# NOAA-OWP/T-Route

Measured on AMD Instinct MI355X. Metric: segment-timesteps/sec, CONUS NHD 2.7M-seg MC, higher is better.
Workload: dtype f32

## Files before the change

include/trmc.h:

```cpp
#ifndef TRMC_H
#define TRMC_H

#include <stddef.h>
#include <stdint.h>

#ifdef __cplusplus
extern "C" {
#endif

#define TRMC_ABI_VERSION 19

typedef enum trmc_status {
    TRMC_OK = 0,
    TRMC_EINVAL = -1,
    TRMC_ECYCLE = -2,
    TRMC_ENODEVICE = -3,
    TRMC_EHIP = -4,
    TRMC_ENOMEM = -5,
    TRMC_ESTATE = -6
} trmc_status;

enum { TRMC_P_DT = 0, TRMC_P_DX, TRMC_P_BW, TRMC_P_TW, TRMC_P_TWCC, TRMC_P_N,
       TRMC_P_NCC, TRMC_P_CS, TRMC_P_S0, TRMC_NPARAM };

// ... 93 lines not shown
                           const uint8_t *cost_hint, int64_t wide_min_rows, int32_t wide_max_levels, int32_t cluster_rows,
                           int64_t *plan_pos_of_row, int32_t *lag_of_row, int32_t *block_of_row, int32_t *wide_levels,
                           int32_t *cluster_levels, int32_t *cluster_blocks);

int trmc_topology_blocks(int64_t nseg, const int64_t *up_ptr, const int64_t *up_idx,
                         const uint8_t *boundary, const uint8_t *cost_hint, int cost_tiers,
                         int64_t *plan_pos_of_row, int32_t *rank_of_row, int32_t *block_rows, int32_t *nblocks);

int trmc_topology_blocks_general(int64_t nseg, const int64_t *up_ptr, const int64_t *up_idx, const uint8_t *boundary,
                                 int32_t stem_min_rows, int64_t *plan_pos_of_row, int32_t *rank_of_row, int32_t *block_rows,
                                 int32_t *nblocks, int32_t *early_blocks, int32_t early_cap, int32_t *nearly);

int trmc_plan_info(const trmc_plan *plan, int64_t *nseg, int64_t *nseg_routed,
                   int32_t *nlevels, int32_t *precision, int32_t *device);
int trmc_plan_lags(const trmc_plan *plan, int32_t *lag_of_row, int32_t *wide_levels, int32_t *cluster_levels);
int trmc_plan_levels(const trmc_plan *plan, int32_t *level_of_row, int64_t *plan_pos_of_row);

int trmc_upload_forcing(trmc_plan *plan, int nsteps, const void *qlat, int64_t nq,
                        const void *q0, const void *boundary_fvd);

int trmc_upload_forcing_packed(trmc_plan *plan, int nsteps, int64_t nq, int64_t nfeat, const int32_t *raw_a,
                               const int32_t *raw_b, const double *pack_a, const double *pack_b,
                               const int64_t *feat_of_row, const void *q0, const void *boundary_fvd);

int trmc_set_boundary_flow_device(trmc_plan *plan, int nsteps, const void *q_dev);

int trmc_set_reservoirs(trmc_plan *plan, int64_t nres, const int64_t *res_rows, const void *par,
                        double routing_period);
int trmc_download_reservoir_inflow(trmc_plan *plan, void *inflow_out);

// ... 114 lines not shown
```

t-route_amd/_lib.py:

```python
import ctypes as C
import os

import numpy as np

_HERE = os.path.dirname(os.path.abspath(__file__))
LIB_PATH = os.environ.get("TRMC_LIB_PATH") or os.path.join(_HERE, "libtrmc.so")

TRMC_OK, TRMC_EINVAL, TRMC_ECYCLE, TRMC_ENODEVICE, TRMC_EHIP, TRMC_ENOMEM, TRMC_ESTATE = 0, -1, -2, -3, -4, -5, -6
ENGINE_AUTO, ENGINE_LEVELS, ENGINE_FLOW, PLAN_SHORT_TS, PLAN_FULL_TS = 0, 1, 2, 4, 8
NPARAM = 9
PARAM_COLS = ("dt", "dx", "bw", "tw", "twcc", "n", "ncc", "cs", "s0")


class Stats(C.Structure):
    _fields_ = [
        ("nseg", C.c_int64), ("nseg_routed", C.c_int64), ("nlevels", C.c_int32), ("nsteps", C.c_int32),
        ("assume_short_ts", C.c_int32), ("main_launches", C.c_int32), ("segment_steps", C.c_int64),
        ("ms_prep", C.c_double), ("ms_main", C.c_double), ("ms_emit", C.c_double), ("ms_total", C.c_double),
        ("wide_levels", C.c_int32), ("wide_k", C.c_int32), ("wide_launches", C.c_int32), ("mid_levels", C.c_int32),
        ("wide_segment_steps", C.c_int64), ("ms_wide", C.c_double), ("mid_k", C.c_int32), ("mid_launches", C.c_int32),
        ("arithmetic", C.c_int32), ("reserved0", C.c_int32),
    ]

    def as_dict(self):
# ... 76 lines not shown
    "trmc_stream_wait": (_int, [_vp, _i64]),
    "trmc_stream_info": (_int, [_vp, _P(_i32), _P(_i32), _P(_i32), _P(_i32), _P(_i32), _P(_i64), _P(_i64), _P(_i64)]),
    "trmc_stream_day_ms": (_int, [_vp, _i64, _P(C.c_double)]),
    "trmc_stream_end": (_int, [_vp]),
    "trmc_plan_arithmetic": (_int, [_vp, _P(_i32)]),
    "trmc_plan_engine": (_int, [_vp, _P(_i32)]),
    "trmc_plan_destroy": (None, [_vp]),
    "trmc_topology_levels": (_int, [_i64, _vp, _vp, _vp, _vp, _vp, _P(_i32)]),
    "trmc_topology_levels_hinted": (_int, [_i64, _vp, _vp, _vp, _vp, _vp, _vp, _P(_i32)]),
    "trmc_topology_clusters": (_int, [_i64, _vp, _vp, _vp, _vp, _i64, _i32, _i32, _vp, _vp, _vp, _P(_i32), _P(_i32), _P(_i32)]),
    "trmc_topology_blocks": (_int, [_i64, _vp, _vp, _vp, _vp, _int, _vp, _vp, _P(_i32), _P(_i32)]),
    "trmc_topology_blocks_general": (_int, [_i64, _vp, _vp, _vp, _i32, _vp, _vp, _P(_i32), _P(_i32), _vp, _i32, _P(_i32)]),
    "trmc_plan_info": (_int, [_vp, _P(_i64), _P(_i64), _P(_i32), _P(_i32), _P(_i32)]),
    "trmc_plan_levels": (_int, [_vp, _vp, _vp]),
    "trmc_plan_lags": (_int, [_vp, _vp, _P(_i32), _P(_i32)]),
    "trmc_upload_forcing": (_int, [_vp, _int, _vp, _i64, _vp, _vp]),
    "trmc_upload_forcing_packed": (_int, [_vp, _int, _i64, _i64, _vp, _vp, _vp, _vp, _vp, _vp, _vp]),
    "trmc_set_boundary_flow_device": (_int, [_vp, _int, _vp]),
    "trmc_set_reservoirs": (_int, [_vp, _i64, _vp, _vp, C.c_double]),
    "trmc_download_reservoir_inflow": (_int, [_vp, _vp]),
    "trmc_set_reservoir_da": (_int, [_vp, _i64, _vp, _vp, _P(ReservoirDaTable), _P(ReservoirDaTable), _P(ReservoirDaTable)]),
    "trmc_download_reservoir_da": (_int, [_vp, _vp, _vp]),
    "trmc_reservoir_da_steps": (_int, [_int, _int, _i64, _i64, _vp, _vp, _vp, _vp, _vp, _vp]),
    "trmc_set_nudging": (_int, [_vp, _int, _i64, _vp, _vp, _vp, _vp]),
    "trmc_set_nudging_successors": (_int, [_vp, C.c_int64, _vp]),
    "trmc_download_nudge": (_int, [_vp, _vp]),
    "trmc_route_device": (_int, [_vp, _int, _int, _int]),
    "trmc_route_begin": (_int, [_vp, _int, _int, _int]),
    "trmc_route_advance": (_int, [_vp, _int]),
    "trmc_route_end": (_int, [_vp]),
# ... 55 lines not shown
    "trmc_event_record": (_int, [_int, _vp, _vp]),
    "trmc_stream_wait_event": (_int, [_int, _vp, _vp]),
}

SIGNATURES_DW = {
    "trdw_last_error": (C.c_char_p, []),
    "trdw_select_device": (_int, [_int]),
    "trdw_diffnw": (_int, [_vp] * 42),
    "trdw_diffnw_batch": (_int, [_int, _vp]),
    "trdw_last_timing": (_int, [_P(C.c_double), _P(C.c_double)]),
    "trdw_configure": (_int, [_vp]),
}

_LIB = None
_HOST_ONLY = {"trmc_last_error", "trmc_abi_version", "trmc_topology_levels", "trmc_topology_levels_hinted", "trmc_topology_blocks", "trmc_topology_clusters",
              "trmc_topology_blocks_general", "trmc_get_stats", "trmc_plan_info", "trmc_plan_levels", "trmc_plan_lags", "trmc_plan_engine",
              "trmc_plan_arithmetic", "trmc_stream_info", "trdw_last_error", "trdw_last_timing", "trdw_configure", "trmc_comm_info"}


class _Marking:

    def __init__(self, cdll):
        self.__dict__["_cdll"] = cdll

    def __getattr__(self, name):
        fn = getattr(self._cdll, name)
        if name in _HOST_ONLY:
            self.__dict__[name] = fn
            return fn

        def call(*args, _fn=fn):
# ... 177 lines not shown
```

t-route_amd/csrc/abi.inc:

```

static void stream_release(trmc_plan *pl);
static bool stream_active(const trmc_plan *pl);

const char *trmc_last_error(void) { return g_err.c_str(); }
int trmc_abi_version(void) { return TRMC_ABI_VERSION; }

int trmc_device_count(int *count)
{
    if (!count) return fail(TRMC_EINVAL, "count is NULL");
    int c = 0;
    hipError_t e = hipGetDeviceCount(&c);
    if (e != hipSuccess) {
        *count = 0;
        return fail(TRMC_ENODEVICE, std::string("hipGetDeviceCount: ") + hipGetErrorString(e));
    }
    *count = c;
    return 0;
}

int trmc_topology_levels(int64_t nseg, const int64_t *up_ptr, const int64_t *up_idx, const uint8_t *boundary,
                         int32_t *level_of_row, int64_t *plan_pos_of_row, int32_t *nlevels)
{
    return trmc_topology_levels_hinted(nseg, up_ptr, up_idx, boundary, nullptr, level_of_row, plan_pos_of_row, nlevels);
}
// ... 6 lines not shown
    const int rc = trmc::build_topology(nseg, up_ptr, up_idx, boundary, t, err, cost_hint);
    if (rc) return fail(rc == -2 ? TRMC_ECYCLE : TRMC_EINVAL, err);
    for (int64_t r = 0; r < nseg; ++r) {
        if (level_of_row) level_of_row[r] = t.level_of_row[r];
        if (plan_pos_of_row) plan_pos_of_row[r] = t.pos_of_row[r];
    }
    if (nlevels) *nlevels = t.nlevels;
    return 0;
}

int trmc_topology_clusters(int64_t nseg, const int64_t *up_ptr, const int64_t *up_idx, const uint8_t *boundary,
                           const uint8_t *cost_hint, int64_t wide_min_rows, int32_t wide_max_levels, int32_t cluster_rows,
                           int64_t *plan_pos_of_row, int32_t *lag_of_row, int32_t *block_of_row, int32_t *wide_levels,
                           int32_t *cluster_levels, int32_t *cluster_blocks)
{
    if (cluster_rows <= 0 || cluster_rows > kTileBlock) return fail(TRMC_EINVAL, "cluster_rows must be in [1, 128]");
    trmc::Topology t;
    std::string err;
    const int rc = trmc::build_topology(nseg, up_ptr, up_idx, boundary, t, err, cost_hint, 0, true, kWideMaxLevels, wide_min_rows,
                                        std::min<int32_t>(wide_max_levels, kWideMaxLevels), 0, 0, 0, cluster_rows);
    if (rc) return fail(rc == -2 ? TRMC_ECYCLE : TRMC_EINVAL, err);
    const int32_t nb = t.ncl > 0 ? (int32_t)t.cblk_ptr.size() - 1 : 0;
    std::vector<int32_t> blk_of_pos((size_t)nseg, -1);
    for (int32_t b = 0; b < nb; ++b)
        for (int32_t p = t.cblk_ptr[(size_t)b]; p < t.cblk_ptr[(size_t)b + 1]; ++p) blk_of_pos[(size_t)p] = b;
    for (int64_t r = 0; r < nseg; ++r) {
        const int32_t p = t.pos_of_row[r];
        if (plan_pos_of_row) plan_pos_of_row[r] = p;
        if (lag_of_row) lag_of_row[r] = t.level_of_row[r] < 0 ? -1 : t.lagk_of_pos[(size_t)p];
        if (block_of_row) block_of_row[r] = blk_of_pos[(size_t)p];
    }
// ... 152 lines not shown
    pl->flow = engine == TRMC_ENGINE_FLOW;
    pl->watchdog_ticks = (uint64_t)(o.flow_watchdog_ms > 0 ? o.flow_watchdog_ms : 30000) * 100000ull;
    {
        int ncu = 256;
        if (hipSetDevice(device) == hipSuccess) (void)hipDeviceGetAttribute(&ncu, hipDeviceAttributeMultiprocessorCount, device);
        trmc_plan::Opt &po = pl->opt;
        po.tol = o.arithmetic == TRMC_ARITH_TOLERANCE;
        po.wide_min_rows = o.wide_min_rows < 0 ? 0 : (o.wide_min_rows > 0 ? o.wide_min_rows : (po.tol ? 256L : 288L) * ncu);
        po.wide_levels = (int32_t)std::min<long>(o.wide_levels > 0 ? o.wide_levels : 16, kWideMaxLevels);
        po.wide_k = o.wide_k > 0 ? o.wide_k : 0;
        po.mid_min_rows = o.mid_min_rows < 0 ? 0 : (o.mid_min_rows > 0 ? o.mid_min_rows : kMidDefaultRowsPerCu * (int64_t)ncu);
        po.mid_levels = (int32_t)std::min<long>(o.mid_levels > 0 ? o.mid_levels : 12, kMidMaxLevels);
        po.mid_k = o.mid_k > 0 ? o.mid_k : 4;
        po.tile_perm_group = o.tile_perm_group < 0 ? 0 : (o.tile_perm_group > 0 ? 1 : -1);
        po.hot_rows = o.hot_rows < 0 ? 0 : (o.hot_rows > 0 ? 1 : -1);
        po.cluster_rows = o.cluster_rows > 0 ? std::min<int32_t>(o.cluster_rows, kTileBlock) : 0;
        po.cluster_late_lag = std::max(0, o.cluster_late_lag);
        po.stream_split = std::max(0, o.stream_split);
        po.hot_wave_rows = std::max(0, std::min(64, o.hot_wave_rows));
        po.velocity_on_demand = o.velocity_on_demand;
        po.sequence = o.sequence_mode != 0;
        po.flow_overlap = o.flow_overlap != 0;
        po.flow_lean = o.flow_lean;
        po.flow_debug = o.flow_debug != 0;
    }
    const bool tiers = (flags & TRMC_PLAN_SHORT_TS) != 0;
    std::string err;
    int64_t wide_min_rows = 0, mid_min_rows = 0;
    int32_t wide_max_levels = 0, mid_max_levels = 0;
    if (tiers && !pl->flow && cost_hint && o.tail_sort >= 0) {
        wide_min_rows = pl->opt.wide_min_rows;
// ... 2 lines not shown
        mid_max_levels = pl->opt.mid_levels;
    }
    int32_t cluster_rows = 0;
    if (tiers && !pl->flow && pl->opt.cluster_rows > 0) {
        cluster_rows = pl->opt.cluster_rows;
        wide_min_rows = pl->opt.wide_min_rows;
        wide_max_levels = pl->opt.wide_levels;
        mid_min_rows = 0;
        mid_max_levels = 0;
        pl->opt.mid_min_rows = 0;
    }
    int32_t stem_min_rows = 0;
    if (pl->flow && (flags & TRMC_PLAN_FULL_TS)) stem_min_rows = o.stem_min_rows < 0 ? 0 : (o.stem_min_rows > 0 ? o.stem_min_rows : 1024);
    const int trc = trmc::build_topology(nseg, up_ptr, up_idx, boundary, pl->topo, err, cost_hint, pl->flow ? kFlowBlock : 0, tiers,
                                         (tiers && !pl->flow) ? kWideMaxLevels : 0, wide_min_rows, wide_max_levels, stem_min_rows,
                                         mid_min_rows, mid_max_levels, cluster_rows, pl->opt.cluster_late_lag);
    if (trc) {
        delete pl;
        return fail(trc == -2 ? TRMC_ECYCLE : TRMC_EINVAL, err);
    }
    pl->device = device;
    pl->hinted = cost_hint != nullptr && (!pl->flow || tiers);
    pl->precision = precision;
    pl->esz = precision == 32 ? 4 : 8;
    pl->nseg = nseg;
    pl->nseg_pad = (nseg + 63) / 64 * 64;
    if (pl->nseg_pad == 0) pl->nseg_pad = 64;
    pl->nrouted = nseg - pl->topo.nboundary;
    pl->dt_uniform = true;
    pl->dt = nseg ? params[TRMC_P_DT] : 0.0;
    for (int64_t r = 1; r < nseg; ++r)
// ... 283 lines not shown
    return 0;
}

int trmc_plan_lags(const trmc_plan *pl, int32_t *lag_of_row, int32_t *wide_levels, int32_t *cluster_levels)
{
    if (!pl) return fail(TRMC_EINVAL, "plan is NULL");
    const trmc::Topology &t = pl->topo;
    if (t.cl_rows <= 0) return fail(TRMC_EINVAL, "the plan is not in cluster order (trmc_plan_options.cluster_rows)");
    for (int64_t r = 0; lag_of_row && r < pl->nseg; ++r)
        lag_of_row[r] = t.level_of_row[r] < 0 ? -1 : t.lagk_of_pos[(size_t)t.pos_of_row[r]];
    if (wide_levels) *wide_levels = t.cl_from_level;
    if (cluster_levels) *cluster_levels = t.ncl;
    return 0;
}

int trmc_plan_levels(const trmc_plan *pl, int32_t *level_of_row, int64_t *plan_pos_of_row)
{
    if (!pl) return fail(TRMC_EINVAL, "plan is NULL");
    for (int64_t r = 0; r < pl->nseg; ++r) {
        if (level_of_row) level_of_row[r] = pl->topo.level_of_row[r];
        if (plan_pos_of_row) plan_pos_of_row[r] = pl->topo.pos_of_row[r];
    }
    return 0;
}

static int final_state_into(trmc_plan *pl, void *dst, int32_t nsteps_of_window)
{
    const int32_t n = (int32_t)pl->nseg, T_ = nsteps_of_window >= 0 ? nsteps_of_window : pl->routed_nsteps;
    const size_t plane = (size_t)(T_ + 1) * pl->nseg_pad;
    const int32_t *rop = (const int32_t *)pl->row_of_pos.p;
// ... 1077 lines not shown
```

t-route_amd/csrc/host_levels.inc:

```

template <class T> T *col(trmc_plan *pl, int c) { return (T *)pl->params.p + (size_t)c * pl->nseg_pad; }

template <class T> int upload_params(trmc_plan *pl, const float *params)
{
    const int64_t n = pl->nseg, np = pl->nseg_pad;
    std::vector<T> host((size_t)TRMC_NPARAM * np, T(0));
    const size_t all_cols = (size_t)kTotalCols * np;
    bool sane = true;
    auto in_range = [](float v) { return v >= 0x1p-14f && v <= 0x1p17f; };
    auto within = [](float v, float lo, float hi) { return v >= lo && v <= hi; };
    for (int64_t p = 0; p < n; ++p) {
        const float *src = params + (size_t)pl->topo.row_of_pos[p] * TRMC_NPARAM;
        for (int c = 0; c < TRMC_NPARAM; ++c) host[(size_t)c * np + p] = (T)src[c];
        const float cs = src[TRMC_P_CS];
        sane = sane && in_range(src[TRMC_P_BW]) && in_range(src[TRMC_P_N]) && (cs == 0.0f || in_range(cs))
               && (src[TRMC_P_TWCC] == 0.0f || in_range(src[TRMC_P_TWCC])) && (src[TRMC_P_NCC] == 0.0f || in_range(src[TRMC_P_NCC]))
               && within(src[TRMC_P_DT], 0x1p-20f, 0x1p40f) && within(src[TRMC_P_DX], 0x1p-10f, 0x1p19f)
               && within(src[TRMC_P_S0], 0x1p-30f, 0x1p10f);
    }
    pl->params_sane = sane && sizeof(T) == 4;
    if (int rc = pl->params.ensure(all_cols * sizeof(T))) return rc;
    HIP_TRY(hipMemcpy(pl->params.p, host.data(), host.size() * sizeof(T), hipMemcpyHostToDevice));
    if (n > 0) {
        hipLaunchKernelGGL((k_make_const<T>), dim3((unsigned)((n + kBlock - 1) / kBlock)), dim3(kBlock), 0, pl->stream,
// ... 146 lines not shown
        }
    }
    if (lazy) {
        if (dec) hipLaunchKernelGGL((k_mc_tile<T, false, true, true>), grid, block, 0, st, a, p0, p1, tile, K);
        else hipLaunchKernelGGL((k_mc_tile<T, false, false, true>), grid, block, 0, st, a, p0, p1, tile, K);
        return;
    }
    if (dec) hipLaunchKernelGGL((k_mc_tile<T, false, true>), grid, block, 0, st, a, p0, p1, tile, K);
    else hipLaunchKernelGGL((k_mc_tile<T, false, false>), grid, block, 0, st, a, p0, p1, tile, K);
}

template <class T>
inline void launch_ctile(hipStream_t st, const StepArgs<T> &a, const int32_t *cblk_ptr, int32_t b0, int32_t b1, int32_t tile, int32_t K,
                         bool tol)
{
    const dim3 grid((unsigned)(b1 - b0)), block(kTileBlock);
    const bool dec = a.dec != nullptr;
    const bool lazy = a.v_every != 0 && !a.out;
    if constexpr (sizeof(T) == 4) {
        if (a.res_da) {
            if (dec) hipLaunchKernelGGL((k_mc_ctile_rda<true>), grid, block, 0, st, a, cblk_ptr, b0, tile, K);
            else hipLaunchKernelGGL((k_mc_ctile_rda<false>), grid, block, 0, st, a, cblk_ptr, b0, tile, K);
            return;
        }
        if (tol) {
            if (lazy) {
                if (dec) hipLaunchKernelGGL((k_mc_ctile<T, true, true, true>), grid, block, 0, st, a, cblk_ptr, b0, tile, K);
                else hipLaunchKernelGGL((k_mc_ctile<T, true, false, true>), grid, block, 0, st, a, cblk_ptr, b0, tile, K);
            } else if (dec) hipLaunchKernelGGL((k_mc_ctile<T, true, true>), grid, block, 0, st, a, cblk_ptr, b0, tile, K);
            else hipLaunchKernelGGL((k_mc_ctile<T, true, false>), grid, block, 0, st, a, cblk_ptr, b0, tile, K);
            return;
// ... 419 lines not shown
```

t-route_amd/csrc/k_mc_ctile.inc:

```
template <class T, bool TOL, bool DEC, bool LAZYV, bool RDA>
__device__ __forceinline__ void mc_ctile_rows(const StepArgs<T> &a, const int32_t *__restrict__ cblk_ptr, int32_t cb0, int32_t tile, int32_t K);
template <class T, bool TOL = false, bool DEC = false, bool LAZYV = false>
__global__ void __launch_bounds__(kTileBlock, sizeof(T) == 4 ? (LAZYV ? TRMC_TILE_WAVES_LAZY : TRMC_TILE_WAVES) : 1)
k_mc_ctile(const StepArgs<T> a, const int32_t *__restrict__ cblk_ptr, const int32_t cb0, const int32_t tile, const int32_t K)
{
    mc_ctile_rows<T, TOL, DEC, LAZYV, false>(a, cblk_ptr, cb0, tile, K);
}
template <bool DEC>
__global__ void __launch_bounds__(kTileBlock, TRMC_TILE_WAVES)
k_mc_ctile_rda(const StepArgs<float> a, const int32_t *__restrict__ cblk_ptr, const int32_t cb0, const int32_t tile, const int32_t K)
{
    mc_ctile_rows<float, false, DEC, false, true>(a, cblk_ptr, cb0, tile, K);
}
template <class T, bool TOL, bool DEC, bool LAZYV, bool RDA>
__device__ __forceinline__ void mc_ctile_rows(const StepArgs<T> &a, const int32_t *__restrict__ cblk_ptr, const int32_t cb0,
                                              const int32_t tile, const int32_t K)
{
    using M = typename DevMath<T, TOL>::type;
    const ColdArgs<StepArgs<T>> cold = cold_args<StepArgs<T>>();
    __shared__ uint64_t s_tab[TRMC_POW_TAB_WORDS];
    __shared__ T s_out[3 * kTileStage * kTileBlock];
    __shared__ T s_x[2 * kTileBlock];
    M m{stage_pow_tables(s_tab), false};
    m.sane = a.sane;

    const int32_t cb = cb0 + (int32_t)blockIdx.x;
    const int32_t lo = cblk_ptr[cb], hi = cblk_ptr[cb + 1];
    int32_t behind, slot, slot_next;
    const bool in_range = seq_locate(a, tile, a.level[lo], behind, slot, slot_next);
    const int32_t t_lo = behind * K + 1, t_hi = min(behind * K + K, a.nsteps);
    if (!in_range || t_lo > t_hi) return;

    int32_t s = lo + (int32_t)threadIdx.x;
    bool active = s < hi;
    if (a.cls_last) {
        const int32_t c = active ? (int32_t)(a.cls_last[s] & 0x7f) : 0x80;
        const int32_t key = (c & 0x80) ? 8 : 7 - min(c, 7);
        bool none;
        s = lo + block_partition_by_class<kTileBlock>(key, none);
        active = !none;
    }
    if (a.cls_last) {
        const int32_t cp = active ? (int32_t)(a.cls_last[s] & 0x7f) : 0;
        if (__any(cp >= 3)) __builtin_amdgcn_s_setprio(3);
        else if (__any(cp == 2)) __builtin_amdgcn_s_setprio(2);
        else __builtin_amdgcn_s_setprio(1);
    } else
        __builtin_amdgcn_s_setprio(2);
    const uint32_t su = (uint32_t)(active ? s : lo);
    const uint32_t sl = su - (uint32_t)lo;
    uint32_t ob = su * (uint32_t)sizeof(T);
    const size_t np = (size_t)a.nseg_pad;
    trmc::ChannelParams<T> p;
    p.dt = a.dt_col ? at(a.dt_col, ob) : a.dt;
// ... 21 lines not shown
    const int32_t in1 = (uy >= lo && uy < hi) ? (uy - lo) * (int32_t)sizeof(T) : -1;
    const int32_t ri = (active && a.res_of_pos) ? a.res_of_pos[su] : -1;
    const int32_t gi = (active && a.gage_of_pos) ? a.gage_of_pos[su] : -1;

    T *const q_tm = a.q_tm + (size_t)slot * (size_t)a.slot_tm;
    const size_t ql_base = (size_t)slot * (size_t)a.slot_qlat;
    T q_prev = at(q_tm + (size_t)(t_lo - 1) * np, ob);
    T d_prev = at(a.d_tm + (size_t)slot * (size_t)a.slot_tm + (size_t)(t_lo - 1) * np, ob);
    T *const out_row = a.out + (size_t)slot * (size_t)a.slot_out + (size_t)a.row_of_pos[su] * (size_t)a.nsteps * 3;
    int32_t ql_col = (t_lo - 1) / a.qts, ql_left = a.qts - (t_lo - 1) % a.qts;
    T ql = at(a.qlat_tm + ql_base + (size_t)ql_col * np, ob);
    m.coef_ok = coef_guard(p.dt, ql);
    const bool count_cost = a.it_sum != nullptr;
    int32_t it_acc = 0, it_last = 0, staged = 0;
    bool over_last = false;
    if (active) s_x[(size_t)((t_lo - 1) & 1) * kTileBlock + sl] = q_prev;
    __syncthreads();
    T *q_up = q_tm + (size_t)(t_lo - 1) * np;
    const int32_t v_every = (LAZYV && DEC) ? cold->v_every : 0;
    int32_t v_left = v_every > 0 ? (v_every - 1) - ((t_lo - 1) % v_every) : 0;
    for (int32_t t = t_lo; t <= t_hi; ++t, q_up += np) {
        bool want_v = false;
        if constexpr (LAZYV && DEC) {
            want_v = v_every > 0 && v_left == 0;
            if (v_every > 0) v_left = v_left == 0 ? v_every - 1 : v_left - 1;
        }
        if (active) {
            if (ql_left == 0) {
                ++ql_col;
                ql = at(cold->qlat_tm + ql_base + (size_t)ql_col * np, ob);
                m.coef_ok = coef_guard(p.dt, ql);
                ql_left = cold->qts;
            }
            --ql_left;
            const T *const sx = s_x + (size_t)((t - 1) & 1) * kTileBlock;
            T qup = T(0);
            if (u.x >= 0) qup += in0 >= 0 ? at(sx, (uint32_t)in0) : at(q_up, (uint32_t)u.x * (uint32_t)sizeof(T));
            if (uy >= 0) qup += in1 >= 0 ? at(sx, (uint32_t)in1) : at(q_up, (uint32_t)uy * (uint32_t)sizeof(T));
            if (uy >= 0) {
                if (u.y & 0x40000000) {
                    const int32_t *const up_ptr = cold->up_ptr, *const up_idx = cold->up_idx;
                    const int32_t k1 = up_ptr[su + 1];
                    for (int32_t k = up_ptr[su] + 2; k < k1; ++k) {
                        const int32_t uk = up_idx[k];
                        qup += (uk >= lo && uk < hi) ? sx[uk - lo] : at(q_up, (uint32_t)uk * (uint32_t)sizeof(T));
                    }
                }
            }
            T q_new, v_new, d_new;
            if (ri >= 0) {
// ... 29 lines not shown
                    const T *const da_a = cold->da_a;
                    const uint8_t mode = cold->da_mode[e];
                    T nudge = T(0);
                    if (mode == 1) {
                        nudge = da_a[e] - q_new;
                        q_new = da_a[e];
                    } else if (mode == 2) {
                        nudge = (da_a[e] - q_new) * cold->da_w[e];
                        q_new = q_new + nudge;
                    }
                    cold->da_nudge[e] = nudge;
                }
            }
            asm volatile("" : "+v"(ob));
            at(q_up + np, ob) = q_new;
            s_x[(size_t)(t & 1) * kTileBlock + sl] = q_new;
            if (t == t_hi) {
                at(cold->d_tm + (size_t)slot * (size_t)cold->slot_tm + (size_t)t * np, ob) = d_new;
                if (cold->seq_slots > 1 && t == cold->nsteps) {
                    at(cold->q_tm + (size_t)slot_next * (size_t)cold->slot_tm, ob) = q_new;
                    at(cold->d_tm + (size_t)slot_next * (size_t)cold->slot_tm, ob) = d_new;
                }
            }
            q_prev = q_new;
            d_prev = d_new;
            if (LAZYV && want_v && it_last > 0) v_new = trmc::step_velocity<T, M>(p, c, d_new, m);
            if (DEC || (!LAZYV && a.out)) {
                T *so = s_out + (size_t)(staged * 3) * kTileBlock + threadIdx.x;
                so[0] = q_new;
                so[kTileBlock] = v_new;
                so[2 * kTileBlock] = d_new;
                ++staged;
                if (staged == kTileStage || t == t_hi) {
                    T *dst = out_row + (size_t)(t - staged) * 3;
                    const T *si = s_out + threadIdx.x;
                    if (LAZYV || !a.out) {
                    } else if (a.out_vec && (staged & 3) == 0) {
                        for (int j = 0; j < 3 * staged / 4; ++j) {
                            float4 v;
                            v.x = (float)si[(4 * j + 0) * kTileBlock];
                            v.y = (float)si[(4 * j + 1) * kTileBlock];
                            v.z = (float)si[(4 * j + 2) * kTileBlock];
                            v.w = (float)si[(4 * j + 3) * kTileBlock];
                            reinterpret_cast<float4 *>(dst)[j] = v;
                        }
                    } else {
                        for (int32_t e = 0; e < 3 * staged; ++e) dst[e] = si[e * kTileBlock];
                    }
                    if constexpr (DEC) {
                        const int32_t ds = cold->dec_stride;
                        for (int32_t k = t / ds; k >= 1 && k * ds > t - staged; --k) {
                            if (k > cold->dec_keep) continue;
                            const int32_t kslot = k * ds - (t - staged) - 1;
                            T *dd = cold->dec + (size_t)slot * (size_t)cold->slot_dec + ((size_t)cold->row_of_pos[su] * (size_t)cold->dec_keep + (size_t)(k - 1)) * 3;
                            dd[0] = si[(kslot * 3 + 0) * kTileBlock];
                            dd[1] = si[(kslot * 3 + 1) * kTileBlock];
                            dd[2] = si[(kslot * 3 + 2) * kTileBlock];
                        }
                    }
                    staged = 0;
                }
            }
        }
        __syncthreads();
    }
    if (!active) return;
    if (t_hi == cold->nsteps) cold->it_prev[su] = (uint8_t)min(it_last, 255);
    if (uint8_t *const cls = cold->cls_last) cls[su] = (uint8_t)(min(it_last, 3) + (over_last ? 4 : 0));
    if (uint16_t *const it_sum = cold->it_sum) it_sum[su] = (uint16_t)min(65535, (int)it_sum[su] + it_acc);
}
```

t-route_amd/csrc/kernels_levels.inc:

```
template <class A> using ColdArgs = const __attribute__((address_space(4))) A *;
template <class A> __device__ __forceinline__ ColdArgs<A> cold_args()
{
    ColdArgs<A> p = (ColdArgs<A>)__builtin_amdgcn_kernarg_segment_ptr();
    asm volatile("" : "+s"(p));
    return p;
}
template <class T> struct StepArgs {
    const T *dx, *bw, *twcc, *n, *ncc, *s0;
    const T *z, *bfd, *sqrt_s0, *sq1pz2, *s0_n, *s0_ncc, *inv_n;
    const T *dt_col;
    T dt;
    const int32_t *up_ptr, *up_idx, *level;
    const int2 *up2;
    const int32_t *lag;
    const T *qlat_tm;
    T *q_tm, *v_tm, *d_tm;
    uint8_t *it_prev;
    uint16_t *it_sum;
    bool sane;
    const int32_t *res_of_pos;
    const T *res_par;
    T *res_inflow;
    T res_dt;
    void *res_da;
// ... 217 lines not shown
    mc_tile_rows<T, TOL, DEC, LAZYV, false>(a, s_begin, s_end, tile, K);
}
template <bool DEC>
__global__ void __launch_bounds__(kTileBlock, TRMC_TILE_WAVES)
k_mc_tile_rda(const StepArgs<float> a, const int32_t s_begin, const int32_t s_end, const int32_t tile, const int32_t K)
{
    mc_tile_rows<float, false, DEC, false, true>(a, s_begin, s_end, tile, K);
}
template <class T, bool TOL, bool DEC, bool LAZYV, bool RDA>
__device__ __forceinline__ void mc_tile_rows(const StepArgs<T> &a, const int32_t s_begin, const int32_t s_end, const int32_t tile,
                                             const int32_t K)
{
    using M = typename DevMath<T, TOL>::type;
    const ColdArgs<StepArgs<T>> cold = cold_args<StepArgs<T>>();
    __shared__ uint64_t s_tab[TRMC_POW_TAB_WORDS];
    __shared__ T s_out[3 * kTileStage * kTileBlock];
    M m{stage_pow_tables(s_tab), false};
    m.sane = a.sane;

    int32_t s;
    bool from_hot = false;
    int32_t *const hot_list = a.cls_last ? cold->hot_list : nullptr;
    const int32_t hot_blocks = hot_list ? cold->hot_home : 0;
    if ((int32_t)blockIdx.x < hot_blocks) {
        const int32_t cur = cold->hot_cur, cap = cold->hot_cap, H = cold->hot_wave_rows;
        const int32_t lane = (int32_t)(threadIdx.x & 63u), wave = (int32_t)blockIdx.x * (kTileBlock / 64) + (int32_t)(threadIdx.x >> 6);
        const int32_t i = wave * H + lane;
        const int32_t nlist = min(cold->hot_cnt[cur], cap);
        if (lane >= H || i >= nlist) return;
        if (lane == 0) atomicAdd(&cold->hot_cnt[3], min(nlist - i, H));
        s = hot_list[(size_t)cur * (size_t)cap + (size_t)i];
// ... 457 lines not shown
```

t-route_amd/csrc/topology.cpp:

```cpp
#include "topology.hpp"

#include <algorithm>
#include <cstdio>
#include <string>
#include <cstdlib>
#include <limits>
#include <utility>

namespace trmc {

int build_topology(int64_t nseg, const int64_t *up_ptr, const int64_t *up_idx,
                   const uint8_t *boundary, Topology &t, std::string &err, const uint8_t *cost_hint, int32_t block_rows,
                   bool cost_tiers, int32_t boundary_floor, int64_t wide_min_rows, int32_t wide_max_levels, int32_t stem_min_rows,
                   int64_t mid_min_rows, int32_t mid_max_levels, int32_t cluster_rows, int32_t cluster_late_lag)
{
    if (nseg < 0 || nseg >= std::numeric_limits<int32_t>::max()) {
        err = "nseg out of range";
        return -1;
    }
    if (nseg > 0 && (!up_ptr || up_ptr[0] != 0)) {
        err = "up_ptr must start at 0";
        return -1;
    }
    const int64_t nnz = nseg ? up_ptr[nseg] : 0;
    for (int64_t r = 0; r < nseg; ++r)
        if (up_ptr[r + 1] < up_ptr[r]) {
            err = "up_ptr is not monotone at row " + std::to_string(r);
            return -1;
        }
// ... 399 lines not shown
            std::stable_sort(idx.begin(), idx.end(), [&](int32_t a, int32_t b) { return key[a] < key[b]; });
            for (int32_t i = 0; i < m; ++i) {
                t.row_of_pos[p0 + i] = rows[idx[i]];
                t.pos_of_row[rows[idx[i]]] = p0 + i;
            }
        }
    }

    if (cluster_rows > 0 && t.nlevels > 0) {
        int32_t W = 0;
        if (wide_min_rows > 0)
            while (W < t.nlevels && W < wide_max_levels && (int64_t)(t.lvl_ptr[W + 1] - t.lvl_ptr[W]) >= wide_min_rows) ++W;
        t.lagk_of_pos.assign(nseg, 0);
        if (W < t.nlevels) {
            const int32_t B = cluster_rows;
            std::vector<int32_t> cl(nseg, -1), root(nseg), size(nseg, 1);
            for (int64_t r = 0; r < nseg; ++r) root[r] = (int32_t)r;
            auto find = [&](int32_t x) {
                while (root[x] != x) {
                    root[x] = root[root[x]];
                    x = root[x];
                }
                return x;
            };
            std::vector<int32_t> tops;
            int32_t maxcl = 0;
            for (const int32_t r : queue) {
                if (t.level_of_row[r] < W) continue;
                int32_t m = -1;
                for (int64_t k = up_ptr[r]; k < up_ptr[r + 1]; ++k) {
// ... 53 lines not shown
            std::vector<std::vector<int32_t>> by_cl((size_t)C);
            for (int32_t c = 0; c < (int32_t)members.size(); ++c) by_cl[(size_t)cl_of[(size_t)c]].push_back(c);
            int32_t p = t.lvl_ptr[W];
            t.cblk_ptr.clear();
            t.cblk_of_cl.assign((size_t)C + 1, 0);
            std::vector<std::vector<int32_t>> bins;
            std::vector<int32_t> fill;
            for (int32_t c = 0; c < C; ++c) {
                std::vector<int32_t> &cs = by_cl[(size_t)c];
                std::stable_sort(cs.begin(), cs.end(), [&](int32_t a, int32_t b) {
                    if (cost_of[(size_t)a] != cost_of[(size_t)b]) return cost_of[(size_t)a] > cost_of[(size_t)b];
                    return members[(size_t)a].size() > members[(size_t)b].size();
                });
                bins.clear();
                fill.clear();
                std::vector<std::vector<int32_t>> by_free((size_t)B + 1);
                for (const int32_t k : cs) {
                    const int32_t n = (int32_t)members[(size_t)k].size();
                    int32_t b = -1;
                    for (int32_t f = n; f <= B && b < 0; ++f)
                        if (!by_free[(size_t)f].empty()) {
                            b = by_free[(size_t)f].back();
                            by_free[(size_t)f].pop_back();
                        }
                    if (b < 0) {
                        b = (int32_t)bins.size();
                        bins.emplace_back();
                        fill.push_back(0);
                    }
                    bins[(size_t)b].push_back(k);
                    fill[(size_t)b] += n;
                    by_free[(size_t)(B - fill[(size_t)b])].push_back(b);
                }
                t.cblk_of_cl[(size_t)c] = (int32_t)t.cblk_ptr.size();
                for (const auto &bin : bins) {
                    t.cblk_ptr.push_back(p);
                    for (const int32_t k : bin)
                        for (const int32_t r : members[(size_t)k]) {
                            t.row_of_pos[p] = r;
                            t.pos_of_row[r] = p;
                            t.lagk_of_pos[p] = W + c;
                            ++p;
                        }
                }
            }
            t.cblk_of_cl[(size_t)C] = (int32_t)t.cblk_ptr.size();
            t.cblk_ptr.push_back(p);
            if (p != t.lvl_ptr[t.nlevels]) {
                err = "internal: the cluster order lost rows";
                return -2;
            }
            t.ncl = C;
            t.tail_from_level = W;
        }
        for (int32_t l = 0; l < W; ++l)
            for (int32_t q = t.lvl_ptr[l]; q < t.lvl_ptr[l + 1]; ++q) t.lagk_of_pos[q] = l;
        t.cl_rows = cluster_rows;
        t.cl_from_level = W;
    } else
    if (cost_hint && wide_min_rows > 0 && wide_max_levels > 0) {
        int32_t W = 0;
        while (W < t.nlevels && W < wide_max_levels && (int64_t)(t.lvl_ptr[W + 1] - t.lvl_ptr[W]) >= wide_min_rows) ++W;
        if (W > 0 && mid_min_rows > 0)
            for (int32_t m = 0; W < t.nlevels && m < mid_max_levels && (int64_t)(t.lvl_ptr[W + 1] - t.lvl_ptr[W]) >= mid_min_rows; ++m) ++W;
        if (W > 0 && W < t.nlevels) {
            const int32_t p0 = t.lvl_ptr[W], p1 = t.lvl_ptr[t.nlevels];
            std::vector<int32_t> rows(t.row_of_pos.begin() + p0, t.row_of_pos.begin() + p1);
            std::stable_sort(rows.begin(), rows.end(), [&](int32_t a, int32_t b) { return cost_hint[a] > cost_hint[b]; });
            for (int32_t i = 0; i < p1 - p0; ++i) {
                t.row_of_pos[p0 + i] = rows[i];
                t.pos_of_row[rows[i]] = p0 + i;
            }
// ... 10 lines not shown
```

t-route_amd/csrc/topology.hpp:

```cpp
#pragma once
#include <cstdint>
#include <string>
#include <vector>

namespace trmc {

struct Topology {
    int64_t nseg = 0;
    int64_t nboundary = 0;
    int32_t nlevels = 0;
    std::vector<int32_t> level_of_row;
    std::vector<int32_t> pos_of_row;
    std::vector<int32_t> row_of_pos;
    std::vector<int32_t> lvl_ptr;
    int32_t tail_from_level = 0;
    std::vector<int32_t> up_ptr;
    std::vector<int32_t> up_idx;
    std::vector<int32_t> boundary_rows;
    int32_t block_rows = 0;
    int32_t nblocks = 0;
    std::vector<int32_t> rank_of_pos;
    int32_t maxrank = 0;
    std::vector<uint8_t> cost_of_wave;
    std::vector<uint8_t> prio_of_wave;
    std::vector<int32_t> early_blocks;
    int32_t cl_rows = 0;
    int32_t cl_from_level = 0;
    int32_t ncl = 0;
    std::vector<int32_t> cblk_ptr;
    std::vector<int32_t> cblk_of_cl;
    std::vector<int32_t> lagk_of_pos;
};

int build_topology(int64_t nseg, const int64_t *up_ptr, const int64_t *up_idx,
                   const uint8_t *boundary, Topology &topo, std::string &err, const uint8_t *cost_hint = nullptr,
                   int32_t block_rows = 0, bool cost_tiers = true, int32_t boundary_floor = 0, int64_t wide_min_rows = 0,
                   int32_t wide_max_levels = 0, int32_t stem_min_rows = 0, int64_t mid_min_rows = 0, int32_t mid_max_levels = 0,
                   int32_t cluster_rows = 0, int32_t cluster_late_lag = 0);

}
```

t-route_amd/plan.py:

```python
import ctypes as C
import os

import numpy as np

from . import _lib


def csr_from_lists(lists):
    ptr = np.zeros(len(lists) + 1, dtype=np.int64)
    if lists:
        ptr[1:] = np.cumsum([len(x) for x in lists])
    idx = np.fromiter((v for x in lists for v in x), dtype=np.int64, count=int(ptr[-1]))
    return ptr, idx


def topology_levels(up_ptr, up_idx, boundary=None, cost_hint=None):
    up_ptr = np.ascontiguousarray(up_ptr, dtype=np.int64)
    up_idx = np.ascontiguousarray(up_idx, dtype=np.int64)
    nseg = up_ptr.shape[0] - 1
    b = None if boundary is None else np.ascontiguousarray(boundary, dtype=np.uint8)
    lvl = np.empty(nseg, dtype=np.int32)
    pos = np.empty(nseg, dtype=np.int64)
    nl = C.c_int32(0)
    h = None if cost_hint is None else np.ascontiguousarray(cost_hint, dtype=np.uint8)
# ... 116 lines not shown
        return {"nseg": nseg.value, "nseg_routed": nr.value, "nlevels": nl.value, "precision": pr.value,
                "device": dev.value}

    def levels(self):
        lvl = np.empty(self.nseg, dtype=np.int32)
        pos = np.empty(self.nseg, dtype=np.int64)
        _lib.check(_lib.lib().trmc_plan_levels(self._h, _lib.ptr(lvl), _lib.ptr(pos)))
        return lvl, pos

    def lags(self):
        lag = np.empty(self.nseg, dtype=np.int32)
        w, c = C.c_int32(0), C.c_int32(0)
        _lib.check(_lib.lib().trmc_plan_lags(self._h, _lib.ptr(lag), C.byref(w), C.byref(c)))
        return lag, w.value, c.value

    def stats(self):
        s = _lib.Stats()
        _lib.check(_lib.lib().trmc_get_stats(self._h, C.byref(s)))
        return s.as_dict()

    def upload_forcing(self, nsteps, qlat, q0, boundary_fvd=None):
        qlat = np.ascontiguousarray(qlat, dtype=self.dtype)
        if qlat.ndim != 2 or qlat.shape[0] != self.nseg:
            raise ValueError(f"Number of rows in Qlat is incorrect: expected ({self.nseg}), got ({qlat.shape[0]})")
        if q0 is not None:
            q0 = np.ascontiguousarray(q0, dtype=self.dtype)
            if q0.shape != (self.nseg, 3):
                raise ValueError("initial_conditions shape mismatch")
        bf = None
        if self.nboundary and boundary_fvd is not None:
# ... 409 lines not shown
```

Measured before the change: 61.76 billion.

## Widen cluster-tile workgroups to pack multiple clusters per block

Decouples the cluster-tile kernel's workgroup size from the generic tile block size. The new size defaults to 512 threads, so the bin packer in topology can place several clusters (each up to 128 rows) into one workgroup. The aim is fewer, fuller blocks and fewer wasted lanes across the cluster-ordered levels. The shared-memory staging depth is halved above 512 threads, and the output staging buffer shrinks to one element when unused (lazy-velocity without decimation). Larger workgroups may lower occupancy and raise barrier cost. A host query for the per-row cluster block assignment is also added.

```diff
diff --git a/include/trmc.h b/include/trmc.h
--- a/include/trmc.h
+++ b/include/trmc.h
@@ -131,6 +131,7 @@
 int trmc_plan_info(const trmc_plan *plan, int64_t *nseg, int64_t *nseg_routed,
                    int32_t *nlevels, int32_t *precision, int32_t *device);
 int trmc_plan_lags(const trmc_plan *plan, int32_t *lag_of_row, int32_t *wide_levels, int32_t *cluster_levels);
+int trmc_plan_cluster_blocks(const trmc_plan *plan, int32_t *block_of_row, int32_t *block_width, int32_t *cluster_blocks);
 int trmc_plan_levels(const trmc_plan *plan, int32_t *level_of_row, int64_t *plan_pos_of_row);
 
 int trmc_upload_forcing(trmc_plan *plan, int nsteps, const void *qlat, int64_t nq,
diff --git a/t-route_amd/_lib.py b/t-route_amd/_lib.py
--- a/t-route_amd/_lib.py
+++ b/t-route_amd/_lib.py
@@ -114,6 +114,7 @@
     "trmc_plan_info": (_int, [_vp, _P(_i64), _P(_i64), _P(_i32), _P(_i32), _P(_i32)]),
     "trmc_plan_levels": (_int, [_vp, _vp, _vp]),
     "trmc_plan_lags": (_int, [_vp, _vp, _P(_i32), _P(_i32)]),
+    "trmc_plan_cluster_blocks": (_int, [_vp, _vp, _P(_i32), _P(_i32)]),
     "trmc_upload_forcing": (_int, [_vp, _int, _vp, _i64, _vp, _vp]),
     "trmc_upload_forcing_packed": (_int, [_vp, _int, _i64, _i64, _vp, _vp, _vp, _vp, _vp, _vp, _vp]),
     "trmc_set_boundary_flow_device": (_int, [_vp, _int, _vp]),
@@ -199,7 +200,7 @@
 
 _LIB = None
 _HOST_ONLY = {"trmc_last_error", "trmc_abi_version", "trmc_topology_levels", "trmc_topology_levels_hinted", "trmc_topology_blocks", "trmc_topology_clusters",
-              "trmc_topology_blocks_general", "trmc_get_stats", "trmc_plan_info", "trmc_plan_levels", "trmc_plan_lags", "trmc_plan_engine",
+              "trmc_topology_blocks_general", "trmc_get_stats", "trmc_plan_info", "trmc_plan_levels", "trmc_plan_lags", "trmc_plan_cluster_blocks", "trmc_plan_engine",
               "trmc_plan_arithmetic", "trmc_stream_info", "trdw_last_error", "trdw_last_timing", "trdw_configure", "trmc_comm_info"}
 
 
diff --git a/t-route_amd/csrc/abi.inc b/t-route_amd/csrc/abi.inc
--- a/t-route_amd/csrc/abi.inc
+++ b/t-route_amd/csrc/abi.inc
@@ -44,7 +44,7 @@
                            int64_t *plan_pos_of_row, int32_t *lag_of_row, int32_t *block_of_row, int32_t *wide_levels,
                            int32_t *cluster_levels, int32_t *cluster_blocks)
 {
-    if (cluster_rows <= 0 || cluster_rows > kTileBlock) return fail(TRMC_EINVAL, "cluster_rows must be in [1, 128]");
+    if (cluster_rows <= 0 || cluster_rows > kClusterRowsMax) return fail(TRMC_EINVAL, "cluster_rows must be in [1, 128]");
     trmc::Topology t;
     std::string err;
     const int rc = trmc::build_topology(nseg, up_ptr, up_idx, boundary, t, err, cost_hint, 0, true, kWideMaxLevels, wide_min_rows,
@@ -227,7 +227,7 @@
         po.mid_k = o.mid_k > 0 ? o.mid_k : 4;
         po.tile_perm_group = o.tile_perm_group < 0 ? 0 : (o.tile_perm_group > 0 ? 1 : -1);
         po.hot_rows = o.hot_rows < 0 ? 0 : (o.hot_rows > 0 ? 1 : -1);
-        po.cluster_rows = o.cluster_rows > 0 ? std::min<int32_t>(o.cluster_rows, kTileBlock) : 0;
+        po.cluster_rows = o.cluster_rows > 0 ? std::min<int32_t>(o.cluster_rows, kClusterRowsMax) : 0;
         po.cluster_late_lag = std::max(0, o.cluster_late_lag);
         po.stream_split = std::max(0, o.stream_split);
         po.hot_wave_rows = std::max(0, std::min(64, o.hot_wave_rows));
@@ -260,7 +260,7 @@
     if (pl->flow && (flags & TRMC_PLAN_FULL_TS)) stem_min_rows = o.stem_min_rows < 0 ? 0 : (o.stem_min_rows > 0 ? o.stem_min_rows : 1024);
     const int trc = trmc::build_topology(nseg, up_ptr, up_idx, boundary, pl->topo, err, cost_hint, pl->flow ? kFlowBlock : 0, tiers,
                                          (tiers && !pl->flow) ? kWideMaxLevels : 0, wide_min_rows, wide_max_levels, stem_min_rows,
-                                         mid_min_rows, mid_max_levels, cluster_rows, pl->opt.cluster_late_lag);
+                                         mid_min_rows, mid_max_levels, cluster_rows, pl->opt.cluster_late_lag, kCtileBlock);
     if (trc) {
         delete pl;
         return fail(trc == -2 ? TRMC_ECYCLE : TRMC_EINVAL, err);
@@ -574,6 +574,22 @@
     return 0;
 }
 
+int trmc_plan_cluster_blocks(const trmc_plan *pl, int32_t *block_of_row, int32_t *block_width, int32_t *cluster_blocks)
+{
+    if (!pl) return fail(TRMC_EINVAL, "plan is NULL");
+    const trmc::Topology &t = pl->topo;
+    if (t.cl_rows <= 0) return fail(TRMC_EINVAL, "the plan is not in cluster order (trmc_plan_options.cluster_rows)");
+    const int32_t nb = t.ncl > 0 ? (int32_t)t.cblk_ptr.size() - 1 : 0;
+    if (block_of_row) {
+        for (int64_t r = 0; r < pl->nseg; ++r) block_of_row[r] = -1;
+        for (int32_t b = 0; b < nb; ++b)
+            for (int32_t p = t.cblk_ptr[(size_t)b]; p < t.cblk_ptr[(size_t)b + 1]; ++p) block_of_row[t.row_of_pos[(size_t)p]] = b;
+    }
+    if (block_width) *block_width = kCtileBlock;
+    if (cluster_blocks) *cluster_blocks = nb;
+    return 0;
+}
+
 int trmc_plan_levels(const trmc_plan *pl, int32_t *level_of_row, int64_t *plan_pos_of_row)
 {
     if (!pl) return fail(TRMC_EINVAL, "plan is NULL");
diff --git a/t-route_amd/csrc/host_levels.inc b/t-route_amd/csrc/host_levels.inc
--- a/t-route_amd/csrc/host_levels.inc
+++ b/t-route_amd/csrc/host_levels.inc
@@ -184,7 +184,7 @@
 inline void launch_ctile(hipStream_t st, const StepArgs<T> &a, const int32_t *cblk_ptr, int32_t b0, int32_t b1, int32_t tile, int32_t K,
                          bool tol)
 {
-    const dim3 grid((unsigned)(b1 - b0)), block(kTileBlock);
+    const dim3 grid((unsigned)(b1 - b0)), block(kCtileBlock);
     const bool dec = a.dec != nullptr;
     const bool lazy = a.v_every != 0 && !a.out;
     if constexpr (sizeof(T) == 4) {
diff --git a/t-route_amd/csrc/k_mc_ctile.inc b/t-route_amd/csrc/k_mc_ctile.inc
--- a/t-route_amd/csrc/k_mc_ctile.inc
+++ b/t-route_amd/csrc/k_mc_ctile.inc
@@ -1,13 +1,21 @@
+#ifndef TRMC_CTILE_BLOCK
+#define TRMC_CTILE_BLOCK 512
+#endif
+constexpr int kCtileBlock = TRMC_CTILE_BLOCK;
+constexpr int kClusterRowsMax = 128;
+static_assert(kCtileBlock % 64 == 0 && kCtileBlock >= kClusterRowsMax && kCtileBlock <= 1024,
+              "TRMC_CTILE_BLOCK: whole wavefronts, at least one cluster, at most one workgroup");
+constexpr int kCtileStage = kCtileBlock > 512 ? kTileStage / 2 : kTileStage;
 template <class T, bool TOL, bool DEC, bool LAZYV, bool RDA>
 __device__ __forceinline__ void mc_ctile_rows(const StepArgs<T> &a, const int32_t *__restrict__ cblk_ptr, int32_t cb0, int32_t tile, int32_t K);
 template <class T, bool TOL = false, bool DEC = false, bool LAZYV = false>
-__global__ void __launch_bounds__(kTileBlock, sizeof(T) == 4 ? (LAZYV ? TRMC_TILE_WAVES_LAZY : TRMC_TILE_WAVES) : 1)
+__global__ void __launch_bounds__(kCtileBlock, sizeof(T) == 4 ? (LAZYV ? TRMC_TILE_WAVES_LAZY : TRMC_TILE_WAVES) : 1)
 k_mc_ctile(const StepArgs<T> a, const int32_t *__restrict__ cblk_ptr, const int32_t cb0, const int32_t tile, const int32_t K)
 {
     mc_ctile_rows<T, TOL, DEC, LAZYV, false>(a, cblk_ptr, cb0, tile, K);
 }
 template <bool DEC>
-__global__ void __launch_bounds__(kTileBlock, TRMC_TILE_WAVES)
+__global__ void __launch_bounds__(kCtileBlock, TRMC_TILE_WAVES)
 k_mc_ctile_rda(const StepArgs<float> a, const int32_t *__restrict__ cblk_ptr, const int32_t cb0, const int32_t tile, const int32_t K)
 {
     mc_ctile_rows<float, false, DEC, false, true>(a, cblk_ptr, cb0, tile, K);
@@ -19,8 +27,8 @@
     using M = typename DevMath<T, TOL>::type;
     const ColdArgs<StepArgs<T>> cold = cold_args<StepArgs<T>>();
     __shared__ uint64_t s_tab[TRMC_POW_TAB_WORDS];
-    __shared__ T s_out[3 * kTileStage * kTileBlock];
-    __shared__ T s_x[2 * kTileBlock];
+    __shared__ T s_out[(DEC || !LAZYV) ? 3 * kCtileStage * kCtileBlock : 1];
+    __shared__ T s_x[2 * kCtileBlock];
     M m{stage_pow_tables(s_tab), false};
     m.sane = a.sane;
 
@@ -37,7 +45,7 @@
         const int32_t c = active ? (int32_t)(a.cls_last[s] & 0x7f) : 0x80;
         const int32_t key = (c & 0x80) ? 8 : 7 - min(c, 7);
         bool none;
-        s = lo + block_partition_by_class<kTileBlock>(key, none);
+        s = lo + block_partition_by_class<kCtileBlock>(key, none);
         active = !none;
     }
     if (a.cls_last) {
@@ -89,7 +97,7 @@
     const bool count_cost = a.it_sum != nullptr;
     int32_t it_acc = 0, it_last = 0, staged = 0;
     bool over_last = false;
-    if (active) s_x[(size_t)((t_lo - 1) & 1) * kTileBlock + sl] = q_prev;
+    if (active) s_x[(size_t)((t_lo - 1) & 1) * kCtileBlock + sl] = q_prev;
     __syncthreads();
     T *q_up = q_tm + (size_t)(t_lo - 1) * np;
     const int32_t v_every = (LAZYV && DEC) ? cold->v_every : 0;
@@ -108,7 +116,7 @@
                 ql_left = cold->qts;
             }
             --ql_left;
-            const T *const sx = s_x + (size_t)((t - 1) & 1) * kTileBlock;
+            const T *const sx = s_x + (size_t)((t - 1) & 1) * kCtileBlock;
             T qup = T(0);
             if (u.x >= 0) qup += in0 >= 0 ? at(sx, (uint32_t)in0) : at(q_up, (uint32_t)u.x * (uint32_t)sizeof(T));
             if (uy >= 0) qup += in1 >= 0 ? at(sx, (uint32_t)in1) : at(q_up, (uint32_t)uy * (uint32_t)sizeof(T));
@@ -168,7 +176,7 @@
             }
             asm volatile("" : "+v"(ob));
             at(q_up + np, ob) = q_new;
-            s_x[(size_t)(t & 1) * kTileBlock + sl] = q_new;
+            s_x[(size_t)(t & 1) * kCtileBlock + sl] = q_new;
             if (t == t_hi) {
                 at(cold->d_tm + (size_t)slot * (size_t)cold->slot_tm + (size_t)t * np, ob) = d_new;
                 if (cold->seq_slots > 1 && t == cold->nsteps) {
@@ -180,26 +188,26 @@
             d_prev = d_new;
             if (LAZYV && want_v && it_last > 0) v_new = trmc::step_velocity<T, M>(p, c, d_new, m);
             if (DEC || (!LAZYV && a.out)) {
-                T *so = s_out + (size_t)(staged * 3) * kTileBlock + threadIdx.x;
+                T *so = s_out + (size_t)(staged * 3) * kCtileBlock + threadIdx.x;
                 so[0] = q_new;
-                so[kTileBlock] = v_new;
-                so[2 * kTileBlock] = d_new;
+                so[kCtileBlock] = v_new;
+                so[2 * kCtileBlock] = d_new;
                 ++staged;
-                if (staged == kTileStage || t == t_hi) {
+                if (staged == kCtileStage || t == t_hi) {
                     T *dst = out_row + (size_t)(t - staged) * 3;
                     const T *si = s_out + threadIdx.x;
                     if (LAZYV || !a.out) {
                     } else if (a.out_vec && (staged & 3) == 0) {
                         for (int j = 0; j < 3 * staged / 4; ++j) {
                             float4 v;
-                            v.x = (float)si[(4 * j + 0) * kTileBlock];
-                            v.y = (float)si[(4 * j + 1) * kTileBlock];
-                            v.z = (float)si[(4 * j + 2) * kTileBlock];
-                            v.w = (float)si[(4 * j + 3) * kTileBlock];
+                            v.x = (float)si[(4 * j + 0) * kCtileBlock];
+                            v.y = (float)si[(4 * j + 1) * kCtileBlock];
+                            v.z = (float)si[(4 * j + 2) * kCtileBlock];
+                            v.w = (float)si[(4 * j + 3) * kCtileBlock];
                             reinterpret_cast<float4 *>(dst)[j] = v;
                         }
                     } else {
-                        for (int32_t e = 0; e < 3 * staged; ++e) dst[e] = si[e * kTileBlock];
+                        for (int32_t e = 0; e < 3 * staged; ++e) dst[e] = si[e * kCtileBlock];
                     }
                     if constexpr (DEC) {
                         const int32_t ds = cold->dec_stride;
@@ -207,9 +215,9 @@
                             if (k > cold->dec_keep) continue;
                             const int32_t kslot = k * ds - (t - staged) - 1;
                             T *dd = cold->dec + (size_t)slot * (size_t)cold->slot_dec + ((size_t)cold->row_of_pos[su] * (size_t)cold->dec_keep + (size_t)(k - 1)) * 3;
-                            dd[0] = si[(kslot * 3 + 0) * kTileBlock];
-                            dd[1] = si[(kslot * 3 + 1) * kTileBlock];
-                            dd[2] = si[(kslot * 3 + 2) * kTileBlock];
+                            dd[0] = si[(kslot * 3 + 0) * kCtileBlock];
+                            dd[1] = si[(kslot * 3 + 1) * kCtileBlock];
+                            dd[2] = si[(kslot * 3 + 2) * kCtileBlock];
                         }
                     }
                     staged = 0;
diff --git a/t-route_amd/csrc/kernels_levels.inc b/t-route_amd/csrc/kernels_levels.inc
--- a/t-route_amd/csrc/kernels_levels.inc
+++ b/t-route_amd/csrc/kernels_levels.inc
@@ -255,7 +255,7 @@
     using M = typename DevMath<T, TOL>::type;
     const ColdArgs<StepArgs<T>> cold = cold_args<StepArgs<T>>();
     __shared__ uint64_t s_tab[TRMC_POW_TAB_WORDS];
-    __shared__ T s_out[3 * kTileStage * kTileBlock];
+    __shared__ T s_out[(DEC || !LAZYV) ? 3 * kTileStage * kTileBlock : 1];
     M m{stage_pow_tables(s_tab), false};
     m.sane = a.sane;
 
diff --git a/t-route_amd/csrc/topology.cpp b/t-route_amd/csrc/topology.cpp
--- a/t-route_amd/csrc/topology.cpp
+++ b/t-route_amd/csrc/topology.cpp
@@ -12,7 +12,8 @@
 int build_topology(int64_t nseg, const int64_t *up_ptr, const int64_t *up_idx,
                    const uint8_t *boundary, Topology &t, std::string &err, const uint8_t *cost_hint, int32_t block_rows,
                    bool cost_tiers, int32_t boundary_floor, int64_t wide_min_rows, int32_t wide_max_levels, int32_t stem_min_rows,
-                   int64_t mid_min_rows, int32_t mid_max_levels, int32_t cluster_rows, int32_t cluster_late_lag)
+                   int64_t mid_min_rows, int32_t mid_max_levels, int32_t cluster_rows, int32_t cluster_late_lag,
+                   int32_t cluster_block_rows)
 {
     if (nseg < 0 || nseg >= std::numeric_limits<int32_t>::max()) {
         err = "nseg out of range";
@@ -442,6 +443,7 @@
         t.lagk_of_pos.assign(nseg, 0);
         if (W < t.nlevels) {
             const int32_t B = cluster_rows;
+            const int32_t BB = std::max(cluster_rows, cluster_block_rows);
             std::vector<int32_t> cl(nseg, -1), root(nseg), size(nseg, 1);
             for (int64_t r = 0; r < nseg; ++r) root[r] = (int32_t)r;
             auto find = [&](int32_t x) {
@@ -525,11 +527,11 @@
                 });
                 bins.clear();
                 fill.clear();
-                std::vector<std::vector<int32_t>> by_free((size_t)B + 1);
+                std::vector<std::vector<int32_t>> by_free((size_t)BB + 1);
                 for (const int32_t k : cs) {
                     const int32_t n = (int32_t)members[(size_t)k].size();
                     int32_t b = -1;
-                    for (int32_t f = n; f <= B && b < 0; ++f)
+                    for (int32_t f = n; f <= BB && b < 0; ++f)
                         if (!by_free[(size_t)f].empty()) {
                             b = by_free[(size_t)f].back();
                             by_free[(size_t)f].pop_back();
@@ -541,7 +543,7 @@
                     }
                     bins[(size_t)b].push_back(k);
                     fill[(size_t)b] += n;
-                    by_free[(size_t)(B - fill[(size_t)b])].push_back(b);
+                    by_free[(size_t)(BB - fill[(size_t)b])].push_back(b);
                 }
                 t.cblk_of_cl[(size_t)c] = (int32_t)t.cblk_ptr.size();
                 for (const auto &bin : bins) {
@@ -567,6 +569,7 @@
         for (int32_t l = 0; l < W; ++l)
             for (int32_t q = t.lvl_ptr[l]; q < t.lvl_ptr[l + 1]; ++q) t.lagk_of_pos[q] = l;
         t.cl_rows = cluster_rows;
+        t.cblk_rows = std::max(cluster_rows, cluster_block_rows);
         t.cl_from_level = W;
     } else
     if (cost_hint && wide_min_rows > 0 && wide_max_levels > 0) {
diff --git a/t-route_amd/csrc/topology.hpp b/t-route_amd/csrc/topology.hpp
--- a/t-route_amd/csrc/topology.hpp
+++ b/t-route_amd/csrc/topology.hpp
@@ -25,6 +25,7 @@
     std::vector<uint8_t> prio_of_wave;
     std::vector<int32_t> early_blocks;
     int32_t cl_rows = 0;
+    int32_t cblk_rows = 0;
     int32_t cl_from_level = 0;
     int32_t ncl = 0;
     std::vector<int32_t> cblk_ptr;
@@ -36,6 +37,6 @@
                    const uint8_t *boundary, Topology &topo, std::string &err, const uint8_t *cost_hint = nullptr,
                    int32_t block_rows = 0, bool cost_tiers = true, int32_t boundary_floor = 0, int64_t wide_min_rows = 0,
                    int32_t wide_max_levels = 0, int32_t stem_min_rows = 0, int64_t mid_min_rows = 0, int32_t mid_max_levels = 0,
-                   int32_t cluster_rows = 0, int32_t cluster_late_lag = 0);
+                   int32_t cluster_rows = 0, int32_t cluster_late_lag = 0, int32_t cluster_block_rows = 0);
 
 }
diff --git a/t-route_amd/plan.py b/t-route_amd/plan.py
--- a/t-route_amd/plan.py
+++ b/t-route_amd/plan.py
@@ -154,6 +154,12 @@
         _lib.check(_lib.lib().trmc_plan_lags(self._h, _lib.ptr(lag), C.byref(w), C.byref(c)))
         return lag, w.value, c.value
 
+    def cluster_blocks(self):
+        blk = np.empty(self.nseg, dtype=np.int32)
+        w, nb = C.c_int32(0), C.c_int32(0)
+        _lib.check(_lib.lib().trmc_plan_cluster_blocks(self._h, _lib.ptr(blk), C.byref(w), C.byref(nb)))
+        return blk, w.value, nb.value
+
     def stats(self):
         s = _lib.Stats()
         _lib.check(_lib.lib().trmc_get_stats(self._h, C.byref(s)))
```

Result: faster. 65.53 billion (median of 6 runs) (+6.1%).
